# leonavery/KSFD

Hardware: AMD Instinct MI355X
Metric: grid-point-updates/sec (implicit step) (higher is better)
Workload: dtype f64

## Files before the change

### ksfd_amd/csrc/spectral.hip.h

```cpp
#pragma once

typedef float2 kcf;
#define KSPEC_MAXSTAGE 7
struct KFFTPlan {
    int n, lg, nstage;
    int m;
    int radix[KSPEC_MAXSTAGE];
    int flags;
    int lgw;
};

__device__ __forceinline__ long long kspec_wt_index(int lgw, int lg_rb, long long ntiles, int nxl, long long tile, int pos, int r)
{
    return lgw < 0 ? ((tile * nxl + pos) << lg_rb) + r
                   : ((((long long)(pos >> lgw) * ntiles + tile) << (lgw + lg_rb)) + ((pos & ((1 << lgw) - 1)) << lg_rb) + r);
}

__device__ __forceinline__ int kspec_ss(const KFFTPlan &P) { const int n2 = 1 << P.lg; return n2 + (n2 >> 4) + 1; }
__device__ __forceinline__ int kspec_sstride(const KFFTPlan &P) { return P.m * kspec_ss(P); }
__device__ __forceinline__ int kspec_lpos(const KFFTPlan &P, int e)
{
    if (P.m == 1) return e + (e >> 4);
    const int b = e >> P.lg, i = e & ((1 << P.lg) - 1);
    return b * kspec_ss(P) + i + (i >> 4);
// ... 173 lines not shown
    KSPEC_LGS_DISPATCH(lg_n - 4, (kspec_stage0_inv_to_t<LGS>(lds, sstride, nseq, tw, st)));
}

template <bool INV>
__device__ __forceinline__ void kspec_stage_any(int radix, kcf *lds, int sstride, int nseq, int lg_n, int lg_L, const kcf *__restrict__ tw)
{
    if (radix == 16) {
        switch (lg_L - 4) {
        case 0: kspec_stage<16, INV, 0>(lds, sstride, nseq, lg_n, tw); break;
        case 1: kspec_stage<16, INV, 1>(lds, sstride, nseq, lg_n, tw); break;
        case 2: kspec_stage<16, INV, 2>(lds, sstride, nseq, lg_n, tw); break;
        case 3: kspec_stage<16, INV, 3>(lds, sstride, nseq, lg_n, tw); break;
        case 4: kspec_stage<16, INV, 4>(lds, sstride, nseq, lg_n, tw); break;
        case 5: kspec_stage<16, INV, 5>(lds, sstride, nseq, lg_n, tw); break;
        case 6: kspec_stage<16, INV, 6>(lds, sstride, nseq, lg_n, tw); break;
        case 7: kspec_stage<16, INV, 7>(lds, sstride, nseq, lg_n, tw); break;
        case 8: kspec_stage<16, INV, 8>(lds, sstride, nseq, lg_n, tw); break;
        case 9: kspec_stage<16, INV, 9>(lds, sstride, nseq, lg_n, tw); break;
        default: kspec_stage<16, INV, 10>(lds, sstride, nseq, lg_n, tw); break;
        }
    }
    else if (radix == 8) { if (lg_L == 3) kspec_stage<8, INV, 0>(lds, sstride, nseq, lg_n, tw); else kspec_stage<8, INV, 2>(lds, sstride, nseq, lg_n, tw); }
    else if (radix == 4) kspec_stage<4, INV, 0>(lds, sstride, nseq, lg_n, tw);
    else kspec_stage<2, INV, 0>(lds, sstride, nseq, lg_n, tw);
}
__device__ __forceinline__ int kspec_lg(int r) { return r == 16 ? 4 : (r == 8 ? 3 : (r == 4 ? 2 : 1)); }

template <bool INV>
__device__ __forceinline__ void kspec_stage3(kcf *lds, int ss, int nseq, int lg, const kcf *__restrict__ tw3)
{
    const float sq = 0.86602540378443865f;
    const int total = nseq << lg;
    for (int item = threadIdx.x; item < total; item += blockDim.x) {
        const int s = item >> lg, i = item & ((1 << lg) - 1);
        kcf *b0 = lds + (long long)s * 3 * ss + i + (i >> 4);
        kcf x0 = b0[0], x1 = b0[ss], x2 = b0[2 * ss];
        kcf w1 = tw3[i];
        if (INV) w1 = kc_conj(w1);
        const kcf w2 = kc_mul(w1, w1);
        if (INV) { x1 = kc_mul(x1, w1); x2 = kc_mul(x2, w2); }
        const kcf t = kc_add(x1, x2), u = kc_sub(x1, x2);
        const kcf a = make_float2(x0.x - 0.5f * t.x, x0.y - 0.5f * t.y);
        const kcf r = INV ? make_float2(-sq * u.y, sq * u.x) : make_float2(sq * u.y, -sq * u.x);
        kcf y1 = kc_add(a, r), y2 = kc_sub(a, r);
        if (!INV) { y1 = kc_mul(y1, w1); y2 = kc_mul(y2, w2); }
        b0[0] = kc_add(x0, t); b0[ss] = y1; b0[2 * ss] = y2;
    }
}

__device__ __forceinline__ void kspec_fft_fwd(const KFFTPlan &P, kcf *lds, int sstride, int nseq, const kcf *__restrict__ tw, int first = 0)
{
    if (P.m == 3) {
        kspec_stage3<false>(lds, kspec_ss(P), nseq, P.lg, tw + (1 << P.lg));
        __syncthreads();
        sstride = kspec_ss(P); nseq *= 3;
    }
    int lg_L = P.lg;
    for (int s = 0; s < first; s++) lg_L -= kspec_lg(P.radix[s]);
    for (int s = first; s < P.nstage; s++) {
        kspec_stage_any<false>(P.radix[s], lds, sstride, nseq, P.lg, lg_L, tw);
        __syncthreads();
        lg_L -= kspec_lg(P.radix[s]);
    }
}
__device__ __forceinline__ void kspec_fft_inv(const KFFTPlan &P, kcf *lds, int sstride, int nseq, const kcf *__restrict__ tw, int last = 0)
{
    const int ss = P.m == 3 ? kspec_ss(P) : sstride, ns = P.m == 3 ? 3 * nseq : nseq;
    int lg_L = 0;
    for (int s = P.nstage - 1; s >= last; s--) {
        lg_L += kspec_lg(P.radix[s]);
        kspec_stage_any<true>(P.radix[s], lds, ss, ns, P.lg, lg_L, tw);
        __syncthreads();
    }
    if (P.m == 3) {
        kspec_stage3<true>(lds, ss, nseq, P.lg, tw + (1 << P.lg));
        __syncthreads();
    }
}

__device__ __forceinline__ int kspec_tile(int b, int ntiles)
{
    return (ntiles & 7) ? b : (b & 7) * (ntiles >> 3) + (b >> 3);
}

template <typename TIN>
__global__ void __launch_bounds__(1024) k_spec_rows_fwd(KFFTPlan PX, int nyp , int rb, int ntiles, int F, const TIN *__restrict__ v, long long plane,
                                                        kcf *__restrict__ W, const kcf *__restrict__ tw, KSpecLin ex)
{
    extern __shared__ kcf kspec_lds[];
    const int nx = PX.n, p = blockIdx.y;
    const int y0 = kspec_tile(blockIdx.x, ntiles < 0 ? -ntiles : ntiles) * rb;
    const int sstride = kspec_sstride(PX);
    const TIN *va = v + (long long)(2 * p) * plane + (long long)y0 * nx;
    const bool has_b = 2 * p + 1 < F;
    const TIN *vb = has_b ? va + plane : va;
    const int half = nx >> 1, lg_half = PX.lg - 1;
    const int lg_rb = 31 - __clz(rb);
    auto row_of = [&](int idx) { return PX.m == 1 ? idx >> lg_half : (idx >> lg_half) / 3; };
    if (sizeof(TIN) == 4 && PX.m == 1 && PX.nstage > 0 && PX.radix[0] == 16 && ex.n == 0 && (PX.flags & 4)) {
        const int S0 = nx >> 4;
        kspec_stage0_fwd_from(kspec_lds, sstride, rb, PX.lg, tw, [&](int r, int i, int q) {
            const TIN *pa = va + (long long)r * nx + i, *pb = vb + (long long)r * nx + i;
            const TIN a = pa[q * S0];
            const TIN b = has_b ? pb[q * S0] : (TIN)0;
            return make_float2((float)a, (float)b);
        });
        __syncthreads();
        kspec_fft_fwd(PX, kspec_lds, sstride, rb, tw, 1);
    } else {
    for (int base = 0; base < rb * half; base += 4 * blockDim.x) {
        double2 a[4], b[4];
#pragma unroll
        for (int u = 0; u < 4; u++) {
            const int idx = base + u * blockDim.x + threadIdx.x;
            a[u] = b[u] = make_double2(0.0, 0.0);
            if (idx < rb * half) {
                const int r = row_of(idx), x = 2 * (idx - r * half);
                a[u] = ksfd_ld2(va + (long long)r * nx + x);
                if (has_b) b[u] = ksfd_ld2(vb + (long long)r * nx + x);
                for (int j = 0; j < ex.n; j++) {
                    const long long o = (long long)(2 * p) * plane + (long long)(y0 + r) * nx + x;
                    const double2 ea = ksfd_ld2(ex.p[j] + o);
                    a[u].x += ex.a[j] * ea.x; a[u].y += ex.a[j] * ea.y;
                    if (has_b) { const double2 eb = ksfd_ld2(ex.p[j] + o + plane); b[u].x += ex.a[j] * eb.x; b[u].y += ex.a[j] * eb.y; }
                }
            }
        }
#pragma unroll
        for (int u = 0; u < 4; u++) {
            const int idx = base + u * blockDim.x + threadIdx.x;
            if (idx < rb * half) {
                const int r = row_of(idx), x = 2 * (idx - r * half);
                kcf *row = kspec_lds + r * sstride;
                row[kspec_lpos(PX, x)] = make_float2((float)a[u].x, (float)b[u].x);
                row[kspec_lpos(PX, x + 1)] = make_float2((float)a[u].y, (float)b[u].y);
            }
        }
    }
    __syncthreads();
    kspec_fft_fwd(PX, kspec_lds, sstride, rb, tw);
    }
    if (ntiles < 0) {
        const long long nt = -ntiles, t = y0 / rb;
        kcf *Wt = W + (long long)p * nt * nx * rb;
        if (PX.lgw < 0) {
            Wt += t * nx * rb;
            for (int idx = threadIdx.x; idx < rb * nx; idx += blockDim.x) {
                const int j = idx >> lg_rb, r = idx & (rb - 1);
                Wt[idx] = kspec_lds[r * sstride + kspec_lpos(PX, j)];
            }
        } else {
            for (int idx = threadIdx.x; idx < rb * nx; idx += blockDim.x) {
                const int j = idx >> lg_rb, r = idx & (rb - 1);
                Wt[kspec_wt_index(PX.lgw, lg_rb, nt, nx, t, j, r)] = kspec_lds[r * sstride + kspec_lpos(PX, j)];
            }
        }
        return;
    }
    kcf *Wp = W + (long long)p * nx * nyp + y0;
    for (int idx = threadIdx.x; idx < rb * nx; idx += blockDim.x) {
        const int j = idx >> lg_rb, r = idx & (rb - 1);
        Wp[(long long)j * nyp + r] = kspec_lds[r * sstride + kspec_lpos(PX, j)];
    }
}

__global__ void __launch_bounds__(1024) k_spec_rows_inv(KFFTPlan PX, int nyp, int rb, int ntiles, int F, const kcf *__restrict__ W,
                                                        double *z, long long plane, const kcf *__restrict__ tw, KSpecLin add)
{
    extern __shared__ kcf kspec_lds[];
    const int nx = PX.n, p = blockIdx.y;
    const int y0 = kspec_tile(blockIdx.x, ntiles) * rb;
    const int sstride = kspec_sstride(PX);
    const kcf *Wp = W + (long long)p * nx * nyp + y0;
    const int lg_rb = 31 - __clz(rb), lg_half = PX.lg - 1;
    const kcf *Wtile = W + ((long long)p * ntiles + y0 / rb) * nx * rb;
    for (int base = 0; base < rb * nx; base += 8 * blockDim.x) {
        kcf t[8];
#pragma unroll
        for (int u = 0; u < 8; u++) {
            const int idx = base + u * blockDim.x + threadIdx.x;
            if (idx < rb * nx) { const int j = idx >> lg_rb, r = idx & (rb - 1); t[u] = (PX.flags & 8) ? Wtile[idx] : Wp[(long long)j * nyp + r]; }
        }
#pragma unroll
        for (int u = 0; u < 8; u++) {
            const int idx = base + u * blockDim.x + threadIdx.x;
            if (idx < rb * nx) { const int j = idx >> lg_rb, r = idx & (rb - 1); kspec_lds[r * sstride + kspec_lpos(PX, j)] = t[u]; }
        }
    }
    __syncthreads();
    const bool has_b = 2 * p + 1 < F;
    const long long o0 = (long long)(2 * p) * plane + (long long)y0 * nx;
    if (PX.m == 1 && PX.nstage > 0 && PX.radix[0] == 16) {
        kspec_fft_inv(PX, kspec_lds, sstride, rb, tw, 1);
        const int S0 = nx >> 4;
        kspec_stage0_inv_to(kspec_lds, sstride, rb, PX.lg, tw, [&](int r, int i, kcf (&c)[16]) {
            const long long o = o0 + (long long)r * nx + i;
#pragma unroll
            for (int hb = 0; hb < 16; hb += 8) {
                double a[8], b[8];
#pragma unroll
                for (int q = 0; q < 8; q++) { a[q] = (double)c[hb + q].x; b[q] = (double)c[hb + q].y; }
#pragma unroll
                for (int j = 0; j < 3; j++)
                    if (j < add.n) {
                        double ta[8], tb[8];
#pragma unroll
                        for (int q = 0; q < 8; q++) { ta[q] = add.p[j][o + (hb + q) * S0]; tb[q] = has_b ? add.p[j][o + (hb + q) * S0 + plane] : 0.0; }
#pragma unroll
                        for (int q = 0; q < 8; q++) { a[q] += add.a[j] * ta[q]; b[q] += add.a[j] * tb[q]; }
                    }
#pragma unroll
                for (int q = 0; q < 8; q++) { z[o + (hb + q) * S0] = a[q]; if (has_b) z[o + (hb + q) * S0 + plane] = b[q]; }
            }
        });
        return;
    }
    kspec_fft_inv(PX, kspec_lds, sstride, rb, tw);
    const int half = nx >> 1;
    for (int idx = threadIdx.x; idx < rb * half; idx += blockDim.x) {
        const int r = PX.m == 1 ? idx >> lg_half : (idx >> lg_half) / 3, x = 2 * (idx - r * half);
        const kcf *row = kspec_lds + r * sstride;
        const kcf c0 = row[kspec_lpos(PX, x)], c1 = row[kspec_lpos(PX, x + 1)];
        const long long o = o0 + (long long)r * nx + x;
        double2 a = make_double2((double)c0.x, (double)c1.x), b = make_double2((double)c0.y, (double)c1.y);
        for (int j = 0; j < add.n; j++) {
            const double2 xa = *reinterpret_cast<const double2 *>(add.p[j] + o);
            a.x += add.a[j] * xa.x; a.y += add.a[j] * xa.y;
            if (has_b) { const double2 xb = *reinterpret_cast<const double2 *>(add.p[j] + o + plane); b.x += add.a[j] * xb.x; b.y += add.a[j] * xb.y; }
        }
        *reinterpret_cast<double2 *>(z + o) = a;
        if (has_b) *reinterpret_cast<double2 *>(z + o + plane) = b;
    }
}

template <int NL>
__device__ __forceinline__ void kspec_symbol(const KSpecSym &S, float L2, kcf (&a)[(NL + 2) / 2], kcf (&b)[(NL + 2) / 2])
{
    constexpr int F = NL + 1, npair = (F + 1) / 2;
    kcf vh[2 * npair];
#pragma unroll
    for (int p = 0; p < npair; p++) {
        const kcf bc = kc_conj(b[p]);
        const kcf su = kc_add(a[p], bc), di = kc_sub(a[p], bc);
        vh[2 * p] = make_float2(0.5f * su.x, 0.5f * su.y);
        vh[2 * p + 1] = make_float2(0.5f * di.y, -0.5f * di.x);
    }
    float den = S.shift - S.a_rr * L2;
    kcf num = vh[0];
    float invd[NL];
#pragma unroll
    for (int l = 0; l < NL; l++) {
        const float d = S.shift + S.gam[l] - S.D[l] * L2;
        invd[l] = __builtin_amdgcn_rcpf(d);
        const float c = S.a_rU[l] * L2 * invd[l];
        den -= c * S.s[l];
        num.x += c * vh[l + 1].x; num.y += c * vh[l + 1].y;
    }
    if (!(fabsf(den) >= S.den_floor)) den = den < 0.0f ? -S.den_floor : S.den_floor;
    const float sc = S.scale * __builtin_amdgcn_rcpf(den);
    kcf zh[2 * npair];
    zh[0] = make_float2(num.x * sc, num.y * sc);
#pragma unroll
    for (int l = 0; l < NL; l++)
        zh[l + 1] = make_float2((vh[l + 1].x * S.scale + S.s[l] * zh[0].x) * invd[l], (vh[l + 1].y * S.scale + S.s[l] * zh[0].y) * invd[l]);
    if (F & 1) zh[F] = make_float2(0.0f, 0.0f);
#pragma unroll
    for (int p = 0; p < npair; p++) {
        const kcf za = zh[2 * p], zb = zh[2 * p + 1];
        a[p] = make_float2(za.x - zb.y, za.y + zb.x);
        b[p] = make_float2(za.x + zb.y, -za.y + zb.x);
    }
}

template <int NL>
__device__ __forceinline__ void kspec_cols_symbol(const KFFTPlan &PY, kcf *lds, int sstride, bool self, int kxA, int kxB, const int *__restrict__ posy,
                                                  const int *__restrict__ kyofpos, const float *__restrict__ lx, const float *__restrict__ ly,
                                                  const int2 *__restrict__ ytab, const KSpecSym &S)
{
    constexpr int F = NL + 1, npair = (F + 1) / 2;
    const int ny = PY.n, half = ny >> 1;
    if (!self) {
        const float lxa = lx[kxA];
        for (int base = threadIdx.x; base < ny; base += 4 * blockDim.x) {
            int2 t[4];
#pragma unroll
            for (int u = 0; u < 4; u++) { const int mpos = base + u * blockDim.x; if (mpos < ny) t[u] = ytab[mpos]; }
#pragma unroll
            for (int u = 0; u < 4; u++) {
                const int mpos = base + u * blockDim.x;
                if (mpos >= ny) break;
                const int m = kspec_lpos(PY, mpos), mp = kspec_lpos(PY, t[u].x);
                const float L2 = lxa + __int_as_float(t[u].y);
                kcf a[npair], b[npair];
#pragma unroll
                for (int p = 0; p < npair; p++) { a[p] = lds[(2 * p) * sstride + m]; b[p] = lds[(2 * p + 1) * sstride + mp]; }
                kspec_symbol<NL>(S, L2, a, b);
#pragma unroll
                for (int p = 0; p < npair; p++) { lds[(2 * p) * sstride + m] = a[p]; lds[(2 * p + 1) * sstride + mp] = b[p]; }
            }
        }
        return;
    }
// ... 470 lines not shown
```

### ksfd_amd/csrc/spectral_host.hip.h

```cpp
#pragma once
#include "spectral_plan.h"

static void spec_free(ksfd_handle *h)
{
    SpecState &S = h->spec;
    void *bufs[] = { S.W, S.W2, S.twx, S.twy, S.twz, S.spos, S.skof, S.ytab, S.pairtab, S.lx, S.ly, S.lz };
    for (void *b : bufs) if (b) hipFree(b);
    S = SpecState();
}

template <typename T> static bool spec_upload(T **dev, const std::vector<T> &host)
{
    return hipMalloc((void **)dev, sizeof(T) * host.size()) == hipSuccess &&
           hipMemcpy(*dev, host.data(), sizeof(T) * host.size(), hipMemcpyHostToDevice) == hipSuccess;
}

static SpecKnobs spec_knobs()
{
    auto num = [](const char *name, int unset) { const char *v = getenv(name); return v ? atoi(v) : unset; };
    static const int diag = num("KSFD_SPEC_DIAG", 0), fuse = num("KSFD_SPEC_FUSE", 7), fuse3 = num("KSFD_SPEC_FUSE3", 3);
    SpecKnobs K;
    K.no3d = getenv("KSFD_SPEC_NO3D");
    K.single = getenv("KSFD_SPEC_SINGLE");
    K.transposed = getenv("KSFD_SPEC_TRANSPOSED");
    K.cz = num("KSFD_SPEC_CZ", K.cz); K.pb = num("KSFD_SPEC_PB", K.pb); K.rb = num("KSFD_SPEC_RB", K.rb);
    K.split = num("KSFD_SPEC_SPLIT", 0);
    K.lgw = num("KSFD_SPEC_LGW", -1);
    K.thr_rows = num("KSFD_SPEC_THRR", 0); K.thr_cols = num("KSFD_SPEC_THRC", 0); K.thr_z = num("KSFD_SPEC_THRZ", 0);
    K.diag = diag; K.fuse = fuse; K.fuse3 = fuse3;
    return K;
}

template <bool R3, bool ONEPIECE> static decltype(&k_spec3_z<0, false>) spec_z_instance(int npair)
{
    return npair == 1 ? k_spec3_z<1, R3, ONEPIECE> : npair == 2 ? k_spec3_z<2, R3, ONEPIECE> : k_spec3_z<0, R3, ONEPIECE>;
}

static void spec_build(ksfd_handle *h)
{
    SpecState &S = h->spec;
    SpecShape &Z = S.shape;
    const KGeom &G = h->G;
    const int P = h->size;
    S.ok = false;
    const SpecKnobs K = spec_knobs();
    if (h->ring && (!h->tr || !h->tr->has_alltoall() || (P != 1 && P != 2 && P != 4 && P != 8) || K.single)) return;
    const SpecGrid I = { G.dim, { h->cfg.n[0], h->cfg.n[1], h->cfg.n[2] }, G.F, P, h->rank, h->ring, G.sloc, G.ng };
    SpecTables T;
    if (!spec_shape(I, K, Z, T)) return;
    const bool d3 = Z.dim == 3;
    S.k_rows_fwd64 = k_spec_rows_fwd<double>;
    S.k_rows_fwd32 = k_spec_rows_fwd<float>;
    S.k_rows_inv = k_spec_rows_inv;
    if (d3) {
        S.k_y_fwd = Z.py.m == 3 ? k_spec3_y_fwd<true> : k_spec3_y_fwd<false>;
        S.k_y_inv = Z.py.m == 3 ? k_spec3_y_inv<true> : k_spec3_y_inv<false>;
        S.k_z = Z.nch == 3 ? spec_z_instance<true, false>(Z.npair) : Z.pz.m == 3 ? spec_z_instance<true, true>(Z.npair) : spec_z_instance<false, false>(Z.npair);
    } else if (Z.cols_split) S.k_cols_split = Z.py.m == 3 ? k_spec_cols_split<true> : k_spec_cols_split<false>;
    else S.k_cols = Z.npair == 1 ? k_spec_cols<1> : Z.npair == 2 ? k_spec_cols<2> : k_spec_cols<0>;
    const struct { const void *kernel; size_t lds; } limits[] = {
        { (const void *)S.k_rows_fwd64, Z.lds_rows }, { (const void *)S.k_rows_fwd32, Z.lds_rows }, { (const void *)S.k_rows_inv, Z.lds_rows },
        { (const void *)S.k_y_fwd, Z.lds_y3 }, { (const void *)S.k_y_inv, Z.lds_y3 }, { (const void *)S.k_z, Z.lds_z3 },
        { (const void *)S.k_cols_split, Z.lds_cols }, { (const void *)S.k_cols, Z.lds_cols } };
    for (const auto &l : limits)
        if (l.kernel && hipFuncSetAttribute(l.kernel, hipFuncAttributeMaxDynamicSharedMemorySize, (int)l.lds) != hipSuccess) { hipGetLastError(); return; }
    const KFFTPlan &ps = d3 ? Z.pz : Z.py;
    const double *ih2 = h->P.inv_h2;
    const size_t wbytes = sizeof(kcf) * Z.welems;
    if (hipMalloc((void **)&S.W, wbytes) != hipSuccess || (Z.need_w2 && hipMalloc((void **)&S.W2, wbytes) != hipSuccess) ||
        !spec_upload(&S.twx, spec_twiddles(Z.px)) || !spec_upload(&S.twy, spec_twiddles(Z.py)) || (d3 && !spec_upload(&S.twz, spec_twiddles(Z.pz))) ||
        !spec_upload(&S.spos, spec_positions(ps)) || !spec_upload(&S.skof, spec_inverse(spec_positions(ps))) || !spec_upload(&S.pairtab, T.pairtab) ||
        !spec_upload(&S.lx, spec_symbol_table(Z.px.n, ih2[0])) || !spec_upload(&S.ly, spec_symbol_table(Z.py.n, ih2[1])) ||
        (d3 && !spec_upload(&S.lz, spec_symbol_table(Z.pz.n, ih2[2]))) ||
        !spec_upload(&S.ytab, spec_partner_table(ps, spec_symbol_table(ps.n, ih2[Z.dim - 1])))) { hipGetLastError(); spec_free(h); return; }
    kcf *back_s = Z.a2a_back_from_w ? S.W : S.W2, *back_r = Z.a2a_back_from_w ? S.W2 : S.W;
    for (const SpecBlock &b : T.a2a_fwd) { S.a2a_fwd_s.push_back({ b.peer, S.W + b.src, b.bytes }); S.a2a_fwd_r.push_back({ b.peer, S.W2 + b.dst, b.bytes }); }
    for (const SpecBlock &b : T.a2a_back) { S.a2a_back_s.push_back({ b.peer, back_s + b.src, b.bytes }); S.a2a_back_r.push_back({ b.peer, back_r + b.dst, b.bytes }); }
    S.ok = true;
}

static int spec_means(ksfd_handle *h)
{
    SpecState &S = h->spec;
    const KGeom &G = h->G;
    const int nb = (int)std::min<long long>((G.nloc + KSFD_BLOCK - 1) / KSFD_BLOCK, 2048);
    {
        Scope sc(h, KC_SPECTRAL, 8.0 * (2 + h->P.nlig) * (double)G.nloc);
        NL_DISPATCH(h->P.nlig, hipLaunchKernelGGL((k_spec_means<NL>), dim3(nb), dim3(KSFD_BLOCK), 0, h->st, G, (const double *)h->coef, h->part));
    }
    HIPCHK(h, hipGetLastError());
    int rc = reduce_rows(h, 1 + h->P.nlig, nb, 0);
    if (rc) return rc;
    const double ntot = (double)h->cfg.n[0] * (double)h->cfg.n[1] * (double)h->cfg.n[2];
    S.a_rr = h->hres[0] / ntot;
    for (int l = 0; l < h->P.nlig; l++) S.a_rU[l] = h->hres[1 + l] / ntot;
    S.means_valid = true;
    return KSFD_OK;
}

struct SpecGuess { int n; const double *Y[3], *b[3]; double c[3]; };

struct SpecRun {
    KSpecSym Y;
    KSpecLin ex, add;
    KFFTPlan px_f, py_c, px_i, py3, pz3;
    long long goff, rows_off, w_off;
    double fn, pn;
    const double *v; const float *v32; double *z;
};

static void spec_rows_fwd(ksfd_handle *h, const SpecRun &R)
{
    const SpecState &S = h->spec;
    const SpecShape &Z = S.shape;
    const KGeom &G = h->G;
    Scope sc(h, KC_SPECTRAL, (R.v32 ? 4.0 : 8.0) * R.fn + 8.0 * R.ex.n * R.fn + R.pn, 8.0 * (1 + R.ex.n) * R.fn);
    const int nt = Z.tile_major ? -Z.ntiles : Z.ntiles;
    for (int c = 0; c < Z.nch; c++) {
        const long long ro = c * R.rows_off;
        kcf *Wf = (Z.tile_major ? S.W2 : S.W) + c * R.w_off;
        KSpecLin exc = R.ex;
        for (int j = 0; j < exc.n; j++) exc.p[j] += ro;
        if (R.v32) hipLaunchKernelGGL(S.k_rows_fwd32, dim3(Z.ntiles, Z.npair), dim3(Z.thr_rows), Z.lds_rows, h->st, R.px_f, Z.nyp, Z.rb, nt, G.F, R.v32 + R.goff + ro, G.plane, Wf, (const kcf *)S.twx, exc);
        else hipLaunchKernelGGL(S.k_rows_fwd64, dim3(Z.ntiles, Z.npair), dim3(Z.thr_rows), Z.lds_rows, h->st, R.px_f, Z.nyp, Z.rb, nt, G.F, R.v + R.goff + ro, G.plane, Wf, (const kcf *)S.twx, exc);
    }
}

static int spec_transpose(ksfd_handle *h, const SpecRun &R, bool back)
{
    SpecState &S = h->spec;
    Scope sc(h, KC_HALO, R.pn);
    if (h->tr->alltoall(back ? S.a2a_back_s : S.a2a_fwd_s, back ? S.a2a_back_r : S.a2a_fwd_r, h->st)) return fail(h, KSFD_ECOMM, "spectral all-to-all failed: %s", h->tr->error().c_str());
    return KSFD_OK;
}

static void spec_cols(ksfd_handle *h, const SpecRun &R)
{
    const SpecState &S = h->spec;
    const SpecShape &Z = S.shape;
    Scope sc(h, KC_SPECTRAL, Z.cols_split == 2 ? (3.0 + 2.0 * Z.npair) * R.pn : Z.cols_split ? (4.0 + Z.npair) * R.pn : 2.0 * R.pn, 0.0);
    const long long pstride = (long long)Z.npair * Z.nxl << Z.lg_pl;
    const kcf *Wt = Z.tile_major ? S.W2 : nullptr;
    const int lg_rb = Z.tile_major ? Z.lg_rb : -1;
    if (!Z.cols_split) {
        hipLaunchKernelGGL(S.k_cols, dim3((unsigned)Z.nblk_cols), dim3(Z.thr_cols), Z.lds_cols, h->st, R.py_c, Z.nxl, Z.lg_pl, pstride, h->ring ? S.W2 : S.W, Wt, lg_rb, (const kcf *)S.twy,
                           (const int4 *)S.pairtab, (const int *)S.spos, (const int *)S.skof, (const float *)S.lx, (const float *)S.ly, (const int2 *)S.ytab, R.Y);
        return;
    }
    kcf *spec = h->ring ? S.W2 : S.W, *res = h->ring ? S.W : S.W2;
    for (int phase = 1; phase <= 2; phase++)
        hipLaunchKernelGGL(S.k_cols_split, dim3((unsigned)Z.nblk_cols, (unsigned)Z.npair, Z.cols_split == 2 ? 2u : 1u), dim3(Z.thr_cols), Z.lds_cols, h->st, phase, R.py_c, Z.nxl, Z.lg_pl, pstride, spec,
                           Wt, lg_rb, res, (const kcf *)S.twy, (const int4 *)S.pairtab, (const int *)S.spos, (const int *)S.skof, (const float *)S.lx, (const float *)S.ly, R.Y);
}

static void spec3_y(ksfd_handle *h, const SpecRun &R, bool inv)
{
    const SpecState &S = h->spec;
    const SpecShape &Z = S.shape;
    const KGeom &G = h->G;
    Scope sc(h, KC_SPECTRAL, 2.0 * R.pn, 0.0);
    const int nzc = (int)(G.sloc / Z.nch);
    const dim3 grid((unsigned)(nzc >> Z.lg_cz), (unsigned)G.nx);
    for (int c = 0; c < Z.nch; c++) {
        if (inv) hipLaunchKernelGGL(S.k_y_inv, grid, dim3(Z.thr_y), Z.lds_y3, h->st, R.py3, (int)G.nx, nzc, Z.lg_cz, Z.npair, (const kcf *)S.W + c * R.w_off, S.W2 + c * R.w_off, (const kcf *)S.twy);
        else hipLaunchKernelGGL(S.k_y_fwd, grid, dim3(Z.thr_y), Z.lds_y3, h->st, R.py3, (int)G.nx, nzc, Z.lg_cz, Z.npair, Z.lg_rb, (const kcf *)S.W2 + c * R.w_off, S.W + c * R.w_off, (const kcf *)S.twy);
    }
}

static void spec3_z(ksfd_handle *h, const SpecRun &R)
{
    const SpecState &S = h->spec;
    const SpecShape &Z = S.shape;
    Scope sc(h, KC_SPECTRAL, 2.0 * R.pn, 0.0);
    const long long ncol = (long long)Z.nxl * Z.py.n, pstride = (long long)Z.npair * ncol << Z.lg_pl;
    hipLaunchKernelGGL(S.k_z, dim3((unsigned)((Z.nent + Z.pb - 1) / Z.pb)), dim3(Z.thr_z), Z.lds_z3, h->st, R.pz3, Z.nent, Z.pb, ncol, Z.lg_pl, pstride, h->ring ? S.W2 : S.W,
                       (const kcf *)S.twz, (const int4 *)S.pairtab, (const int *)S.spos, (const int *)S.skof, (const float *)S.lx, (const float *)S.ly, (const float *)S.lz, (const int2 *)S.ytab, R.Y);
}

static void spec_rows_inv(ksfd_handle *h, const SpecRun &R)
{
    const SpecState &S = h->spec;
    const SpecShape &Z = S.shape;
    const KGeom &G = h->G;
    Scope sc(h, KC_SPECTRAL, R.pn + 8.0 * (1 + R.add.n) * R.fn, 8.0 * (1 + R.add.n) * R.fn);
    const kcf *Wi = (Z.dim == 3 || Z.cols_split) ? S.W2 : S.W;
    for (int c = 0; c < Z.nch; c++) {
        const long long ro = c * R.rows_off;
        KSpecLin addc = R.add;
        for (int j = 0; j < addc.n; j++) addc.p[j] += ro;
        hipLaunchKernelGGL(S.k_rows_inv, dim3(Z.ntiles, Z.npair), dim3(Z.thr_rows), Z.lds_rows, h->st, R.px_i, Z.nyp, Z.rb, Z.ntiles, G.F, Wi + c * R.w_off, R.z + R.goff + ro, G.plane, (const kcf *)S.twx, addc);
    }
}

static int spec_apply(ksfd_handle *h, double shift, const double *v, double *z, const double *xadd = nullptr, const float *v32 = nullptr, const SpecGuess *guess = nullptr)
{
    SpecState &S = h->spec;
    const SpecShape &Z = S.shape;
    const KGeom &G = h->G;
    if (!S.ok || !S.means_valid) return fail(h, KSFD_EINVAL, "spectral preconditioner not available for this handle");
    SpecRun R;
    memset(&R, 0, sizeof R);
    R.v = v; R.v32 = v32; R.z = z;
    R.Y.nlig = h->P.nlig;
    R.Y.shift = (float)shift; R.Y.a_rr = (float)S.a_rr;
    R.Y.scale = (float)(1.0 / ((double)G.nx * (double)h->cfg.n[1] * (double)h->cfg.n[2]));
    R.Y.den_floor = (float)(0.02 * shift);
    for (int l = 0; l < h->P.nlig; l++) { R.Y.a_rU[l] = (float)S.a_rU[l]; R.Y.s[l] = (float)h->P.lig_s[l]; R.Y.gam[l] = (float)h->P.lig_gamma[l]; R.Y.D[l] = (float)h->P.lig_D[l]; }
    R.goff = (long long)G.ng * G.inner;
    R.rows_off = G.sloc / Z.nch * G.inner;
    R.w_off = (long long)Z.npair * G.nx * Z.nyp;
    if (xadd) { R.add.n = 1; R.add.p[0] = xadd + R.goff; R.add.a[0] = 1.0; }
    if (guess && !v32) {
        for (int j = 0; j < guess->n && j < 3; j++) {
            R.ex.p[R.ex.n] = guess->b[j] + R.goff; R.ex.a[R.ex.n++] = -guess->c[j];
            R.add.p[R.add.n] = guess->Y[j] + R.goff; R.add.a[R.add.n++] = guess->c[j];
        }
    }
    R.px_f = R.px_i = Z.px; R.py_c = R.py3 = Z.py; R.pz3 = Z.pz;
    if (Z.diag & 1) R.px_f.nstage = 0;
    if (Z.diag & 2) R.py_c.nstage = 0;
    if (Z.diag & 4) R.px_i.nstage = 0;
    R.px_f.flags = R.py_c.flags = R.px_i.flags = Z.fuse;
    R.px_f.lgw = R.py_c.lgw = Z.lgw;
    R.py3.flags = R.pz3.flags = Z.fuse3;
    R.fn = (double)G.F * (double)G.nloc; R.pn = 8.0 * Z.npair * (double)G.nloc;
    const bool d3 = Z.dim == 3;
    int rc;
    spec_rows_fwd(h, R);
    if (d3) spec3_y(h, R, false);
    if (h->ring && (rc = spec_transpose(h, R, false))) return rc;
    if (d3) spec3_z(h, R); else spec_cols(h, R);
    if (h->ring && (rc = spec_transpose(h, R, true))) return rc;
    if (d3) spec3_y(h, R, true);
    spec_rows_inv(h, R);
    HIPCHK(h, hipGetLastError());
    return KSFD_OK;
}
```

### ksfd_amd/csrc/spectral_plan.h

```cpp
#pragma once
#include <limits.h>
#include <math.h>
#include <string.h>
#include <algorithm>
#include <vector>

#ifndef __HIP__
struct int4 { int x, y, z, w; };
static int4 make_int4(int x, int y, int z, int w) { int4 r = { x, y, z, w }; return r; }
#endif

static int spec_log2(long long v) { int lg = 0; while ((1LL << lg) < v) lg++; return lg; }

static bool spec_plan(long long n, KFFTPlan &P)
{
    int m = 1;
    long long n2 = n;
    if (n2 > 0 && n2 % 3 == 0) { m = 3; n2 /= 3; }
    if (n2 < (m == 3 ? 16 : 32) || n2 > (m == 3 ? 4096 : 16384) || (n2 & (n2 - 1))) return false;
    const int lg = spec_log2(n2);
    P.n = (int)n; P.lg = lg; P.m = m; P.nstage = 0; P.flags = 0; P.lgw = -1;
    int left = lg;
    if (lg == 5) { P.radix[P.nstage++] = 16; P.radix[P.nstage++] = 2; left = 0; }
    while (left >= 4 && left != 5 && P.nstage < KSPEC_MAXSTAGE) { P.radix[P.nstage++] = 16; left -= 4; }
// ... 26 lines not shown
static bool spec_ownership(const KFFTPlan &Q, int P, SpecOwn &O)
{
    if ((P != 1 && P != 2 && P != 4 && P != 8) || Q.nstage < 1 || Q.radix[0] != 16) return false;
    O.P = P; O.npiece = 16 * Q.m; O.w = Q.n / O.npiece; O.per = O.npiece / P;
    for (int o = 0; o < 16; o++) O.piece[o] = spec_digit_order[o];
    if (Q.m == 3) for (int d = 0; d < 16; d++) { O.piece[16 + 2 * d] = 16 + d; O.piece[17 + 2 * d] = 32 + 15 - d; }
    for (int o = 0; o < O.npiece; o++) O.order[O.piece[o]] = o;
    return true;
}
static int spec_owner(const SpecOwn &O, int pos) { return O.order[pos / O.w] / O.per; }
static int spec_local_index(const SpecOwn &O, int pos) { return (O.order[pos / O.w] % O.per) * O.w + pos % O.w; }
static int spec_piece_start(const SpecOwn &O, int rank, int i) { return O.piece[rank * O.per + i] * O.w; }

static bool spec_slab_eligible(const KFFTPlan &px, const KFFTPlan &py, int P, long long nyl, SpecOwn &O, int &nch)
{
    if (!spec_ownership(px, P, O)) return false;
    nch = py.m;
    if (nyl < 4 || nyl % nch) return false;
    const long long cs = nyl / nch;
    return cs >= 2 && !(cs & (cs - 1));
}
static size_t spec_a2a_src(const SpecOwn &O, int nx, int npair, long long cs, int peer, int p, int i, int c)
{
    return (((size_t)c * npair + p) * nx + spec_piece_start(O, peer, i)) * cs;
}
static size_t spec_a2a_dst(const SpecOwn &O, int npair, int nch, long long cs, int sender, int p, int i, int c)
{
    return ((((size_t)sender * nch + c) * npair + p) * ((size_t)O.per * O.w) + (size_t)i * O.w) * cs;
}

static bool spec_slab3_eligible(const KFFTPlan &px, const KFFTPlan &pz, int P, long long nzl, SpecOwn &O, int &nch)
{
    if (!spec_ownership(px, P, O)) return false;
    nch = pz.m;
    if (nzl < 2 || nzl * P != pz.n || nzl % nch) return false;
    const long long cs = nzl / nch;
    return cs >= 2 && !(cs & (cs - 1));
}
static size_t spec_a2a3_src(const SpecOwn &O, int nx, int ny, int npair, long long cs, int peer, int p, int i, int c)
{
    return spec_a2a_src(O, nx, npair, ny * cs, peer, p, i, c);
}
static size_t spec_a2a3_dst(const SpecOwn &O, int ny, int npair, int nch, long long cs, int sender, int p, int i, int c)
{
    return spec_a2a_dst(O, npair, nch, ny * cs, sender, p, i, c);
}

static std::vector<kcf> spec_twiddles(const KFFTPlan &P)
{
    const int n2 = 1 << P.lg;
    std::vector<kcf> t((size_t)n2 * (P.m == 3 ? 2 : 1));
    for (int k = 0; k < n2; k++) { const double a = -2.0 * M_PI * k / n2; t[k] = make_float2((float)cos(a), (float)sin(a)); }
    if (P.m == 3) for (int k = 0; k < n2; k++) { const double a = -2.0 * M_PI * k / P.n; t[n2 + k] = make_float2((float)cos(a), (float)sin(a)); }
    return t;
}
static std::vector<int> spec_positions(const KFFTPlan &Q) { std::vector<int> p(Q.n); for (int k = 0; k < Q.n; k++) p[k] = spec_pos(Q, k); return p; }
static std::vector<int> spec_inverse(const std::vector<int> &p) { std::vector<int> q(p.size()); for (size_t k = 0; k < p.size(); k++) q[p[k]] = (int)k; return q; }
static std::vector<int2> spec_partner_table(const KFFTPlan &Q, const std::vector<float> &l)
{
    const std::vector<int> pos = spec_positions(Q), kof = spec_inverse(pos);
    std::vector<int2> t(Q.n);
    for (int m = 0; m < Q.n; m++) {
        const int k = kof[m];
        int bits;
        memcpy(&bits, &l[k], sizeof bits);
        t[m] = make_int2(pos[(Q.n - k) % Q.n], bits);
    }
    return t;
}
static std::vector<float> spec_symbol_table(int n, double inv_h2)
{
    std::vector<float> l(n);
    for (int k = 0; k < n; k++) { const double th = 2.0 * M_PI * k / n; l[k] = (float)((-30.0 + 32.0 * cos(th) - 2.0 * cos(2.0 * th)) / 12.0 * inv_h2); }
    return l;
}

struct SpecKnobs {
    bool no3d = false, single = false, transposed = false;
    int cz = INT_MAX, pb = INT_MAX, rb = INT_MAX;
    int split = 0;
    int lgw = -1;
    int thr_rows = 0, thr_cols = 0, thr_z = 0;
    int diag = 0, fuse = 7, fuse3 = 3;
};
struct SpecGrid {
    int dim;
    long long n[3];
    int F, P, rank;
    bool ring;
    long long sloc;
    int ng;
};
struct SpecShape {
    int dim = 2, npair = 0;
    KFFTPlan px, py, pz;
    int nch = 1;
    int rb = 0, lg_rb = 0, ntiles = 0;
    int nyp = 0;
    int nxl = 0, lg_pl = 0;
    int cols_split = 0;
    bool tile_major = false, need_w2 = false;
    bool a2a_back_from_w = false;
    int lgw = -1;
    int lg_cz = 0, pb = 1;
    int nent = 0, nblk_cols = 0;
    size_t lds_rows = 0, lds_cols = 0, lds_y3 = 0, lds_z3 = 0;
    size_t welems = 0;
    int thr_rows = 0, thr_cols = 0, thr_y = 0, thr_z = 0;
    int diag = 0, fuse = 0, fuse3 = 0;
};
struct SpecBlock { int peer; size_t src, dst, bytes; };
struct SpecTables {
    std::vector<int4> pairtab;
    std::vector<SpecBlock> a2a_fwd, a2a_back;
};

static bool spec_shape(const SpecGrid &I, const SpecKnobs &K, SpecShape &S, SpecTables &T)
{
    S = SpecShape();
    T = SpecTables();
    const bool d3 = I.dim == 3, ring = I.ring;
    if ((I.dim != 2 && !d3) || (d3 && (K.no3d || (!ring && I.ng != 0)))) return false;
    const long long nsl = I.sloc;
    if (!spec_plan(I.n[0], S.px) || !spec_plan(I.n[1], S.py) || (d3 && !spec_plan(I.n[2], S.pz))) return false;
    const int nx = S.px.n, ny = S.py.n;
    SpecOwn O;
    int nch = 1;
    if (ring && !(d3 ? spec_slab3_eligible(S.px, S.pz, I.P, nsl, O, nch) : spec_slab_eligible(S.px, S.py, I.P, nsl, O, nch))) return false;
    if (d3 ? (S.px.radix[0] != 16 || nx > 32768 || ny > 32768 || nsl < 2) : nsl < 4) return false;
    const long long cs = nsl / nch;
    const long long crows = d3 ? ny * cs : cs;
    S.dim = I.dim;
    S.nch = nch;
    S.npair = (I.F + 1) / 2;
    const size_t lds_max = 160 * 1024 - 1024, row_bytes = sizeof(kcf) * spec_sstride(S.px);
    int rb = 16;
    if (d3) {
        while (rb > 1 && row_bytes * rb > lds_max) rb >>= 1;
        while (rb > 2 && crows / rb < 512) rb >>= 1;
        if (row_bytes * rb > lds_max || crows % rb || ny % rb) return false;
    } else {
        rb = (int)std::min<size_t>(lds_max / row_bytes, 16);
        while (rb & (rb - 1)) rb &= rb - 1;
        while (rb > 1 && (nsl % rb)) rb >>= 1;
        if (rb < 1) return false;
        while (rb > 2 && nsl / rb < 512) rb >>= 1;
        rb = std::max(1, std::min(rb, K.rb));
    }
    S.rb = rb;
    S.lg_rb = spec_log2(rb);
    S.ntiles = (int)(crows / rb);
    S.lds_rows = row_bytes * rb;
    S.thr_rows = K.thr_rows > 0 ? K.thr_rows : (int)std::min<long long>(1024, std::max<long long>(256, (long long)rb * nx / 16));
    S.nxl = nx / I.P;
    S.lg_pl = spec_log2(cs);
    S.diag = K.diag;
    S.fuse3 = K.fuse3 & 3;
    if (d3) {
        const size_t ycol = sizeof(kcf) * spec_sstride(S.py) * S.npair, zcol = sizeof(kcf) * spec_sstride(S.pz) * 2 * S.npair;
        int cz = 16, pb = 16;
        while (cz > 1 && (ycol * cz > lds_max / 2 || cs % cz)) cz >>= 1;
        cz = std::max(1, std::min(cz, K.cz));
        while (pb > 1 && zcol * pb > lds_max / 8) pb >>= 1;
        pb = std::max(1, std::min(pb, K.pb));
        if (ycol * cz > lds_max || zcol * pb > lds_max) return false;
        S.lg_cz = spec_log2(cz);
        S.pb = pb;
        S.lds_y3 = ycol * cz;
        S.lds_z3 = zcol * pb;
        S.thr_y = (int)std::min<long long>(1024, std::max<long long>(256, ((long long)S.npair * cz * ny / 16 + 63) & ~63LL));
        S.thr_z = K.thr_z > 0 ? K.thr_z : (int)std::min<long long>(1024, std::max<long long>(128, ((long long)2 * S.npair * pb * S.pz.n / 16 + 63) & ~63LL));
        S.nyp = (int)crows;
        S.tile_major = S.need_w2 = true;
        S.fuse = K.fuse & 7;
    } else {
        const size_t col = sizeof(kcf) * spec_sstride(S.py);
        S.lds_cols = col * 2 * S.npair;
        S.cols_split = (S.lds_cols > lds_max || (K.split == 1 && S.npair > 1) || K.split == 2) ? 1 : 0;
        if (S.cols_split) S.lds_cols = col * 2;
        if (S.cols_split && (S.lds_cols > lds_max || K.split == 2)) {
            S.cols_split = 2;
            S.lds_cols = col;
        }
        if (S.lds_cols > lds_max) return false;
        S.thr_cols = K.thr_cols > 0 ? K.thr_cols
                                    : (int)std::min<long long>(512, std::max<long long>(128, (long long)(S.cols_split == 2 ? 1 : 2) * (S.cols_split ? 1 : S.npair) * ny / 16));
        S.nyp = (int)(ring ? cs : 1LL << S.lg_pl);
        S.tile_major = !ring && rb >= 2 && !K.transposed;
        S.need_w2 = ring || S.tile_major || S.cols_split;
        if (S.tile_major) S.lgw = std::max(-1, std::min(K.lgw, 8));
        if (S.lgw >= 0 && (S.nxl & ((1 << S.lgw) - 1))) S.lgw = -1;
        S.fuse = (ring || S.cols_split || !S.tile_major) ? (K.fuse & 7) : K.fuse;
    }
    S.welems = (size_t)S.npair * nx * S.nyp * nch;
    auto mine = [&](int j) { return !ring || spec_owner(O, j) == I.rank; };
    auto local_index = [&](int j) { return !ring ? j : spec_local_index(O, j); };
    const std::vector<int> posx = spec_positions(S.px), posy = spec_positions(S.py);
    for (int kx = 0; kx <= nx / 2; kx++) {
        const int kxm = (nx - kx) % nx, ja = local_index(posx[kx]), jb = local_index(posx[kxm]);
        if (!mine(posx[kx])) continue;
        if (!d3) {
            if (kx == 0) T.pairtab.push_back(make_int4(ja, local_index(posx[nx / 2]), 0, nx / 2 + 1));
            else if (kx != nx / 2) T.pairtab.push_back(make_int4(ja, jb, kx, 0));
        } else for (int ky = 0; ky < ny; ky++) {
            const int kym = (ny - ky) % ny;
            const bool self = kxm == kx && kym == ky;
            if (!self && (kxm < kx || (kxm == kx && kym < ky))) continue;
            T.pairtab.push_back(make_int4(ja * ny + posy[ky], jb * ny + posy[kym], kx | (ky << 16), self ? 1 : 0));
        }
    }
    std::sort(T.pairtab.begin(), T.pairtab.end(), [](const int4 &a, const int4 &b) { return a.x < b.x; });
    (d3 ? S.nent : S.nblk_cols) = (int)T.pairtab.size();
    if (!d3 && S.nblk_cols != S.nxl / 2) return false;
    if (ring) {
        const long long ce = d3 ? ny * cs : cs;
        const size_t bytes = sizeof(kcf) * (size_t)O.w * ce;
        for (int q = 0; q < I.P; q++)
            for (int p = 0; p < S.npair; p++)
                for (int i = 0; i < O.per; i++) for (int c = 0; c < nch; c++) {
                    const size_t mine_for_q = spec_a2a_src(O, nx, S.npair, ce, q, p, i, c);
                    const size_t from_q = spec_a2a_dst(O, S.npair, nch, ce, q, p, i, c);
                    T.a2a_fwd.push_back({ q, mine_for_q, from_q, bytes });
                    T.a2a_back.push_back({ q, from_q, mine_for_q, bytes });
                }
        S.a2a_back_from_w = S.cols_split != 0;
    }
    return true;
}
```

Measured before the change: 1.798 billion.

## Split row-FFT tiles into half-height sub-tiles to double LDS occupancy

Result: slower. 1.752 billion (-2.5%).

```diff
diff --git a/ksfd_amd/csrc/spectral.hip.h b/ksfd_amd/csrc/spectral.hip.h
--- a/ksfd_amd/csrc/spectral.hip.h
+++ b/ksfd_amd/csrc/spectral.hip.h
@@ -279,6 +279,14 @@
 {
     return (ntiles & 7) ? b : (b & 7) * (ntiles >> 3) + (b >> 3);
 }
+__device__ __forceinline__ int kspec_subtile(int ntiles, int rb, int &tile, int &r0)
+{
+    const int lg_sub = 31 - __clz((int)gridDim.x / ntiles);
+    const int lb = kspec_tile(blockIdx.x, gridDim.x);
+    tile = lb >> lg_sub;
+    r0 = (lb & ((1 << lg_sub) - 1)) * (rb >> lg_sub);
+    return rb >> lg_sub;
+}
 
 template <typename TIN>
 __global__ void __launch_bounds__(1024) k_spec_rows_fwd(KFFTPlan PX, int nyp , int rb, int ntiles, int F, const TIN *__restrict__ v, long long plane,
@@ -286,37 +294,39 @@
 {
     extern __shared__ kcf kspec_lds[];
     const int nx = PX.n, p = blockIdx.y;
-    const int y0 = kspec_tile(blockIdx.x, ntiles < 0 ? -ntiles : ntiles) * rb;
+    int tile, r0;
+    const int rbk = kspec_subtile(ntiles < 0 ? -ntiles : ntiles, rb, tile, r0);
+    const int y0 = tile * rb, yb = y0 + r0;
     const int sstride = kspec_sstride(PX);
-    const TIN *va = v + (long long)(2 * p) * plane + (long long)y0 * nx;
+    const TIN *va = v + (long long)(2 * p) * plane + (long long)yb * nx;
     const bool has_b = 2 * p + 1 < F;
     const TIN *vb = has_b ? va + plane : va;
     const int half = nx >> 1, lg_half = PX.lg - 1;
-    const int lg_rb = 31 - __clz(rb);
+    const int lg_rb = 31 - __clz(rb), lg_rbk = 31 - __clz(rbk);
     auto row_of = [&](int idx) { return PX.m == 1 ? idx >> lg_half : (idx >> lg_half) / 3; };
     if (sizeof(TIN) == 4 && PX.m == 1 && PX.nstage > 0 && PX.radix[0] == 16 && ex.n == 0 && (PX.flags & 4)) {
         const int S0 = nx >> 4;
-        kspec_stage0_fwd_from(kspec_lds, sstride, rb, PX.lg, tw, [&](int r, int i, int q) {
+        kspec_stage0_fwd_from(kspec_lds, sstride, rbk, PX.lg, tw, [&](int r, int i, int q) {
             const TIN *pa = va + (long long)r * nx + i, *pb = vb + (long long)r * nx + i;
             const TIN a = pa[q * S0];
             const TIN b = has_b ? pb[q * S0] : (TIN)0;
             return make_float2((float)a, (float)b);
         });
         __syncthreads();
-        kspec_fft_fwd(PX, kspec_lds, sstride, rb, tw, 1);
+        kspec_fft_fwd(PX, kspec_lds, sstride, rbk, tw, 1);
     } else {
-    for (int base = 0; base < rb * half; base += 4 * blockDim.x) {
+    for (int base = 0; base < rbk * half; base += 4 * blockDim.x) {
         double2 a[4], b[4];
 #pragma unroll
         for (int u = 0; u < 4; u++) {
             const int idx = base + u * blockDim.x + threadIdx.x;
             a[u] = b[u] = make_double2(0.0, 0.0);
-            if (idx < rb * half) {
+            if (idx < rbk * half) {
                 const int r = row_of(idx), x = 2 * (idx - r * half);
                 a[u] = ksfd_ld2(va + (long long)r * nx + x);
                 if (has_b) b[u] = ksfd_ld2(vb + (long long)r * nx + x);
                 for (int j = 0; j < ex.n; j++) {
-                    const long long o = (long long)(2 * p) * plane + (long long)(y0 + r) * nx + x;
+                    const long long o = (long long)(2 * p) * plane + (long long)(yb + r) * nx + x;
                     const double2 ea = ksfd_ld2(ex.p[j] + o);
                     a[u].x += ex.a[j] * ea.x; a[u].y += ex.a[j] * ea.y;
                     if (has_b) { const double2 eb = ksfd_ld2(ex.p[j] + o + plane); b[u].x += ex.a[j] * eb.x; b[u].y += ex.a[j] * eb.y; }
@@ -326,7 +336,7 @@
 #pragma unroll
         for (int u = 0; u < 4; u++) {
             const int idx = base + u * blockDim.x + threadIdx.x;
-            if (idx < rb * half) {
+            if (idx < rbk * half) {
                 const int r = row_of(idx), x = 2 * (idx - r * half);
                 kcf *row = kspec_lds + r * sstride;
                 row[kspec_lpos(PX, x)] = make_float2((float)a[u].x, (float)b[u].x);
@@ -335,28 +345,28 @@
         }
     }
     __syncthreads();
-    kspec_fft_fwd(PX, kspec_lds, sstride, rb, tw);
+    kspec_fft_fwd(PX, kspec_lds, sstride, rbk, tw);
     }
     if (ntiles < 0) {
-        const long long nt = -ntiles, t = y0 / rb;
+        const long long nt = -ntiles, t = tile;
         kcf *Wt = W + (long long)p * nt * nx * rb;
         if (PX.lgw < 0) {
             Wt += t * nx * rb;
-            for (int idx = threadIdx.x; idx < rb * nx; idx += blockDim.x) {
-                const int j = idx >> lg_rb, r = idx & (rb - 1);
-                Wt[idx] = kspec_lds[r * sstride + kspec_lpos(PX, j)];
+            for (int idx = threadIdx.x; idx < rbk * nx; idx += blockDim.x) {
+                const int j = idx >> lg_rbk, r = idx & (rbk - 1);
+                Wt[(j << lg_rb) + r0 + r] = kspec_lds[r * sstride + kspec_lpos(PX, j)];
             }
         } else {
-            for (int idx = threadIdx.x; idx < rb * nx; idx += blockDim.x) {
-                const int j = idx >> lg_rb, r = idx & (rb - 1);
-                Wt[kspec_wt_index(PX.lgw, lg_rb, nt, nx, t, j, r)] = kspec_lds[r * sstride + kspec_lpos(PX, j)];
+            for (int idx = threadIdx.x; idx < rbk * nx; idx += blockDim.x) {
+                const int j = idx >> lg_rbk, r = idx & (rbk - 1);
+                Wt[kspec_wt_index(PX.lgw, lg_rb, nt, nx, t, j, r0 + r)] = kspec_lds[r * sstride + kspec_lpos(PX, j)];
             }
         }
         return;
     }
-    kcf *Wp = W + (long long)p * nx * nyp + y0;
-    for (int idx = threadIdx.x; idx < rb * nx; idx += blockDim.x) {
-        const int j = idx >> lg_rb, r = idx & (rb - 1);
+    kcf *Wp = W + (long long)p * nx * nyp + yb;
+    for (int idx = threadIdx.x; idx < rbk * nx; idx += blockDim.x) {
+        const int j = idx >> lg_rbk, r = idx & (rbk - 1);
         Wp[(long long)j * nyp + r] = kspec_lds[r * sstride + kspec_lpos(PX, j)];
     }
 }
@@ -366,31 +376,33 @@
 {
     extern __shared__ kcf kspec_lds[];
     const int nx = PX.n, p = blockIdx.y;
-    const int y0 = kspec_tile(blockIdx.x, ntiles) * rb;
+    int tile, r0;
+    const int rbk = kspec_subtile(ntiles, rb, tile, r0);
+    const int yb = tile * rb + r0;
     const int sstride = kspec_sstride(PX);
-    const kcf *Wp = W + (long long)p * nx * nyp + y0;
-    const int lg_rb = 31 - __clz(rb), lg_half = PX.lg - 1;
-    const kcf *Wtile = W + ((long long)p * ntiles + y0 / rb) * nx * rb;
-    for (int base = 0; base < rb * nx; base += 8 * blockDim.x) {
+    const kcf *Wp = W + (long long)p * nx * nyp + yb;
+    const int lg_rb = 31 - __clz(rb), lg_rbk = 31 - __clz(rbk), lg_half = PX.lg - 1;
+    const kcf *Wtile = W + ((long long)p * ntiles + tile) * nx * rb + r0;
+    for (int base = 0; base < rbk * nx; base += 8 * blockDim.x) {
         kcf t[8];
 #pragma unroll
         for (int u = 0; u < 8; u++) {
             const int idx = base + u * blockDim.x + threadIdx.x;
-            if (idx < rb * nx) { const int j = idx >> lg_rb, r = idx & (rb - 1); t[u] = (PX.flags & 8) ? Wtile[idx] : Wp[(long long)j * nyp + r]; }
+            if (idx < rbk * nx) { const int j = idx >> lg_rbk, r = idx & (rbk - 1); t[u] = (PX.flags & 8) ? Wtile[(j << lg_rb) + r] : Wp[(long long)j * nyp + r]; }
         }
 #pragma unroll
         for (int u = 0; u < 8; u++) {
             const int idx = base + u * blockDim.x + threadIdx.x;
-            if (idx < rb * nx) { const int j = idx >> lg_rb, r = idx & (rb - 1); kspec_lds[r * sstride + kspec_lpos(PX, j)] = t[u]; }
+            if (idx < rbk * nx) { const int j = idx >> lg_rbk, r = idx & (rbk - 1); kspec_lds[r * sstride + kspec_lpos(PX, j)] = t[u]; }
         }
     }
     __syncthreads();
     const bool has_b = 2 * p + 1 < F;
-    const long long o0 = (long long)(2 * p) * plane + (long long)y0 * nx;
+    const long long o0 = (long long)(2 * p) * plane + (long long)yb * nx;
     if (PX.m == 1 && PX.nstage > 0 && PX.radix[0] == 16) {
-        kspec_fft_inv(PX, kspec_lds, sstride, rb, tw, 1);
+        kspec_fft_inv(PX, kspec_lds, sstride, rbk, tw, 1);
         const int S0 = nx >> 4;
-        kspec_stage0_inv_to(kspec_lds, sstride, rb, PX.lg, tw, [&](int r, int i, kcf (&c)[16]) {
+        kspec_stage0_inv_to(kspec_lds, sstride, rbk, PX.lg, tw, [&](int r, int i, kcf (&c)[16]) {
             const long long o = o0 + (long long)r * nx + i;
 #pragma unroll
             for (int hb = 0; hb < 16; hb += 8) {
@@ -412,9 +424,9 @@
         });
         return;
     }
-    kspec_fft_inv(PX, kspec_lds, sstride, rb, tw);
+    kspec_fft_inv(PX, kspec_lds, sstride, rbk, tw);
     const int half = nx >> 1;
-    for (int idx = threadIdx.x; idx < rb * half; idx += blockDim.x) {
+    for (int idx = threadIdx.x; idx < rbk * half; idx += blockDim.x) {
         const int r = PX.m == 1 ? idx >> lg_half : (idx >> lg_half) / 3, x = 2 * (idx - r * half);
         const kcf *row = kspec_lds + r * sstride;
         const kcf c0 = row[kspec_lpos(PX, x)], c1 = row[kspec_lpos(PX, x + 1)];
diff --git a/ksfd_amd/csrc/spectral_host.hip.h b/ksfd_amd/csrc/spectral_host.hip.h
--- a/ksfd_amd/csrc/spectral_host.hip.h
+++ b/ksfd_amd/csrc/spectral_host.hip.h
@@ -27,6 +27,7 @@
     K.split = num("KSFD_SPEC_SPLIT", 0);
     K.lgw = num("KSFD_SPEC_LGW", -1);
     K.thr_rows = num("KSFD_SPEC_THRR", 0); K.thr_cols = num("KSFD_SPEC_THRC", 0); K.thr_z = num("KSFD_SPEC_THRZ", 0);
+    K.half = num("KSFD_SPEC_HALF", -1);
     K.diag = diag; K.fuse = fuse; K.fuse3 = fuse3;
     return K;
 }
@@ -109,6 +110,13 @@
     const double *v; const float *v32; double *z;
 };
 
+struct SpecRowLaunch { unsigned nblk, thr; size_t lds; };
+static SpecRowLaunch spec_row_launch(const SpecShape &Z, int kernel)
+{
+    if (Z.half & kernel) return { (unsigned)(Z.ntiles * (Z.rb / Z.rbk)), (unsigned)Z.thr_rows_blk, Z.lds_rows_blk };
+    return { (unsigned)Z.ntiles, (unsigned)Z.thr_rows, Z.lds_rows };
+}
+
 static void spec_rows_fwd(ksfd_handle *h, const SpecRun &R)
 {
     const SpecState &S = h->spec;
@@ -116,13 +124,14 @@
     const KGeom &G = h->G;
     Scope sc(h, KC_SPECTRAL, (R.v32 ? 4.0 : 8.0) * R.fn + 8.0 * R.ex.n * R.fn + R.pn, 8.0 * (1 + R.ex.n) * R.fn);
     const int nt = Z.tile_major ? -Z.ntiles : Z.ntiles;
+    const SpecRowLaunch L = spec_row_launch(Z, R.v32 ? SPEC_HALF_FWD32 : SPEC_HALF_FWD64);
     for (int c = 0; c < Z.nch; c++) {
         const long long ro = c * R.rows_off;
         kcf *Wf = (Z.tile_major ? S.W2 : S.W) + c * R.w_off;
         KSpecLin exc = R.ex;
         for (int j = 0; j < exc.n; j++) exc.p[j] += ro;
-        if (R.v32) hipLaunchKernelGGL(S.k_rows_fwd32, dim3(Z.ntiles, Z.npair), dim3(Z.thr_rows), Z.lds_rows, h->st, R.px_f, Z.nyp, Z.rb, nt, G.F, R.v32 + R.goff + ro, G.plane, Wf, (const kcf *)S.twx, exc);
-        else hipLaunchKernelGGL(S.k_rows_fwd64, dim3(Z.ntiles, Z.npair), dim3(Z.thr_rows), Z.lds_rows, h->st, R.px_f, Z.nyp, Z.rb, nt, G.F, R.v + R.goff + ro, G.plane, Wf, (const kcf *)S.twx, exc);
+        if (R.v32) hipLaunchKernelGGL(S.k_rows_fwd32, dim3(L.nblk, Z.npair), dim3(L.thr), L.lds, h->st, R.px_f, Z.nyp, Z.rb, nt, G.F, R.v32 + R.goff + ro, G.plane, Wf, (const kcf *)S.twx, exc);
+        else hipLaunchKernelGGL(S.k_rows_fwd64, dim3(L.nblk, Z.npair), dim3(L.thr), L.lds, h->st, R.px_f, Z.nyp, Z.rb, nt, G.F, R.v + R.goff + ro, G.plane, Wf, (const kcf *)S.twx, exc);
     }
 }
 
@@ -184,11 +193,12 @@
     const KGeom &G = h->G;
     Scope sc(h, KC_SPECTRAL, R.pn + 8.0 * (1 + R.add.n) * R.fn, 8.0 * (1 + R.add.n) * R.fn);
     const kcf *Wi = (Z.dim == 3 || Z.cols_split) ? S.W2 : S.W;
+    const SpecRowLaunch L = spec_row_launch(Z, SPEC_HALF_INV);
     for (int c = 0; c < Z.nch; c++) {
         const long long ro = c * R.rows_off;
         KSpecLin addc = R.add;
         for (int j = 0; j < addc.n; j++) addc.p[j] += ro;
-        hipLaunchKernelGGL(S.k_rows_inv, dim3(Z.ntiles, Z.npair), dim3(Z.thr_rows), Z.lds_rows, h->st, R.px_i, Z.nyp, Z.rb, Z.ntiles, G.F, Wi + c * R.w_off, R.z + R.goff + ro, G.plane, (const kcf *)S.twx, addc);
+        hipLaunchKernelGGL(S.k_rows_inv, dim3(L.nblk, Z.npair), dim3(L.thr), L.lds, h->st, R.px_i, Z.nyp, Z.rb, Z.ntiles, G.F, Wi + c * R.w_off, R.z + R.goff + ro, G.plane, (const kcf *)S.twx, addc);
     }
 }
 
diff --git a/ksfd_amd/csrc/spectral_plan.h b/ksfd_amd/csrc/spectral_plan.h
--- a/ksfd_amd/csrc/spectral_plan.h
+++ b/ksfd_amd/csrc/spectral_plan.h
@@ -132,6 +132,7 @@
     int lgw = -1;
     int thr_rows = 0, thr_cols = 0, thr_z = 0;
     int diag = 0, fuse = 7, fuse3 = 3;
+    int half = -1;
 };
 struct SpecGrid {
     int dim;
@@ -146,6 +147,9 @@
     KFFTPlan px, py, pz;
     int nch = 1;
     int rb = 0, lg_rb = 0, ntiles = 0;
+    int rbk = 0, thr_rows_blk = 0;
+    size_t lds_rows_blk = 0;
+    int half = 0;
     int nyp = 0;
     int nxl = 0, lg_pl = 0;
     int cols_split = 0;
@@ -159,6 +163,8 @@
     int thr_rows = 0, thr_cols = 0, thr_y = 0, thr_z = 0;
     int diag = 0, fuse = 0, fuse3 = 0;
 };
+enum { SPEC_HALF_FWD32 = 1, SPEC_HALF_FWD64 = 2, SPEC_HALF_INV = 4, SPEC_HALF_ALL = 7 };
+#define SPEC_HALF_DEFAULT (SPEC_HALF_FWD32 | SPEC_HALF_FWD64)
 struct SpecBlock { int peer; size_t src, dst, bytes; };
 struct SpecTables {
     std::vector<int4> pairtab;
@@ -202,6 +208,14 @@
     S.ntiles = (int)(crows / rb);
     S.lds_rows = row_bytes * rb;
     S.thr_rows = K.thr_rows > 0 ? K.thr_rows : (int)std::min<long long>(1024, std::max<long long>(256, (long long)rb * nx / 16));
+    S.rbk = rb; S.lds_rows_blk = S.lds_rows; S.thr_rows_blk = S.thr_rows; S.half = 0;
+    if (rb >= 2 && 2 * (row_bytes * (rb / 2)) <= lds_max) {
+        const long long bfly = (long long)(rb / 2) * nx / 16;
+        const int thr = K.thr_rows > 0 ? K.thr_rows : (int)std::min<long long>(1024, std::max<long long>(256, bfly));
+        const bool pays = !d3 && !ring && S.px.m == 1 && S.lds_rows > lds_max / 2 && bfly >= thr;
+        S.half = K.half >= 0 ? (K.half & SPEC_HALF_ALL) : (pays ? SPEC_HALF_DEFAULT : 0);
+        if (S.half) { S.rbk = rb / 2; S.lds_rows_blk = row_bytes * S.rbk; S.thr_rows_blk = thr; }
+    }
     S.nxl = nx / I.P;
     S.lg_pl = spec_log2(cs);
     S.diag = K.diag;
```
